# ChocoWu/SeTok

Hardware: AMD Instinct MI355X
Metric: images/s SeTok encode (ViT-L/14, 224^2, dyn-k) (higher is better)
Workload: dtype bf16; 1 GPU; cfg2: ViT-L/14 224^2 (24 of 24 layers, select_layer=-1 as the reference's launch scripts pass it), dyn-k DPC-kNN (k=64, threshold=0.125), SeTok head 1024/2 heads/ff 4096 -> 4096, mm_in_projector mlp2x_gelu; encode-only; batch_per_gpu=256, global_batch=256, slowest_rank=0

## Files before the change

### setok_amd/csrc/common.h

```cpp
#pragma once
#include <hip/hip_runtime.h>
#include <stdint.h>
#include <stdio.h>
#include <stdarg.h>

#include "../../include/setok_hip.h"

#ifdef SETOK_HALF
typedef _Float16 bf16;
typedef __attribute__((ext_vector_type(8))) _Float16 bf16x8;
typedef __attribute__((ext_vector_type(4))) _Float16 bf16x4;
typedef __attribute__((ext_vector_type(2))) _Float16 bf16x2;
#define SETOK_BF16 SETOK_F16
#define __builtin_amdgcn_mfma_f32_16x16x32_bf16 __builtin_amdgcn_mfma_f32_16x16x32_f16
#define __builtin_amdgcn_mfma_f32_32x32x16_bf16 __builtin_amdgcn_mfma_f32_32x32x16_f16
#else
typedef __bf16 bf16;
typedef __attribute__((ext_vector_type(8))) __bf16 bf16x8;
typedef __attribute__((ext_vector_type(4))) __bf16 bf16x4;
typedef __attribute__((ext_vector_type(2))) __bf16 bf16x2;
#endif
typedef __attribute__((ext_vector_type(4))) float f32x4;
typedef __attribute__((ext_vector_type(16))) float f32x16;

// ... 128 lines not shown
    return v;
}

__device__ inline float gelu_erf_fast(float x) {
    const float z = fabsf(x) * 0.70710678118654752440f;
    const float t = __builtin_amdgcn_rcpf(fmaf(0.3275911f, z, 1.0f));
    const float poly = t * fmaf(t, fmaf(t, fmaf(t, fmaf(t, 1.061405429f, -1.453152027f), 1.421413741f), -0.284496736f), 0.254829592f);
    const float half_tail = 0.5f * poly * __builtin_amdgcn_exp2f(-z * z * 1.44269504088896340736f);
    return x * (x >= 0.f ? 1.0f - half_tail : half_tail);
}

__device__ inline unsigned long long dropout_word(unsigned long long seed, unsigned long long group) {
    unsigned long long z = seed + group * 0x9E3779B97F4A7C15ull;
    z = (z ^ (z >> 30)) * 0xBF58476D1CE4E5B9ull;
    z = (z ^ (z >> 27)) * 0x94D049BB133111EBull;
    z ^= z >> 31;
    return z;
}
__device__ inline bool dropout_keep(unsigned long long seed, unsigned long long ctr, unsigned thresh16) {
    return (unsigned)((dropout_word(seed, ctr >> 2) >> (16 * (unsigned)(ctr & 3))) & 0xffffu) >= thresh16;
}


#ifdef SETOK_HALF
__device__ inline void split2(float x, bf16& hi, bf16& lo) {
    hi = (bf16)x;
    lo = (bf16)(x - (float)hi);
}
#else
__device__ inline void split2(float x, bf16& hi, bf16& lo) {
    const unsigned u = __builtin_bit_cast(unsigned, x);
    hi = __builtin_bit_cast(bf16, (unsigned short)(u >> 16));
    const float r = x - __builtin_bit_cast(float, u & 0xffff0000u);
    lo = __builtin_bit_cast(bf16, (unsigned short)(__builtin_bit_cast(unsigned, r) >> 16));
}
#endif
__device__ inline bf16x8 ln_col_frag(float c, float b) {
    bf16x8 f;
#pragma unroll
    for (int e = 0; e < 8; ++e) f[e] = (bf16)0.0f;
    {
        bf16 ch, cl, bh, bl;
        split2(c, ch, cl); split2(b, bh, bl);
        f[0] = ch; f[1] = ch; f[2] = cl; f[3] = cl; f[4] = bh; f[5] = bh; f[6] = bl; f[7] = bl;
    }
    return f;
}
__device__ inline bf16x8 ln_row_frag(float mean, float rstd) {
    bf16x8 f;
#pragma unroll
    for (int e = 0; e < 8; ++e) f[e] = (bf16)0.0f;
    {
        bf16 mh, ml, sh, sl;
        split2(-mean, mh, ml); split2(1.0f / rstd, sh, sl);
        f[0] = mh; f[1] = ml; f[2] = mh; f[3] = ml; f[4] = sh; f[5] = sl; f[6] = sh; f[7] = sl;
    }
    return f;
}

template <typename T>
__device__ inline T swiglu16(float gate, float up) {
    const float g = (float)(T)gate, u = (float)(T)up;
    float s;
    if constexpr (sizeof(T) == 4) s = g / (1.0f + expf(-g));
    else s = g * __builtin_amdgcn_rcpf(1.0f + __builtin_amdgcn_exp2f(-1.44269504088896340736f * g));
    return (T)((float)(T)s * u);
}
constexpr int SETOK_ACT_SWIGLU_PAIRS = 100;

__device__ inline float act_apply(float v, int act) {
    if (act == SETOK_ACT_QUICK_GELU) return v / (1.0f + expf(-1.702f * v));
    if (act == SETOK_ACT_GELU_ERF) return 0.5f * v * (1.0f + erff(v * 0.70710678118654752440f));
    if (act == SETOK_ACT_SILU) return v / (1.0f + expf(-v));
    return v;
}
```

### setok_amd/csrc/gemm_persist.hip

```cpp
#include "lds_mma.h"
#include <stdlib.h>
#include <type_traits>

namespace {

constexpr int TM = 256, TK = 64;
constexpr int STAGE = 64 * 1024;
constexpr int BOFF = TM * TK * 2;

struct PArgs {
    const bf16* A; const bf16* W; const float* bias; const bf16* res; bf16* C;
    int64_t lda, ldc;
    int M, N, K, tilesM, tilesN;
    const float* zero_bias;
    float* Cf;
    int64_t sA, sW, sC;
    int nbatch;
    const float* ln_stats;
    const float* ln_colsum;
    const int32_t* m_dev;
    int rem_rows;
    int rem_tiles;
    int rem_shape;
};

__device__ inline void s_barrier_lgkm() {
    asm volatile("s_waitcnt lgkmcnt(0)\n\ts_barrier" ::: "memory");
}

__device__ inline int swz(int row) { return (row >> 1) & 7; }
typedef __attribute__((ext_vector_type(4))) float f32x4;

__device__ inline bf16x8 ln_frag_lane(const f32x4 raw, int g4) {
    f32x4 v = raw;
    if (g4 != 0) { v[0] = 0.f; v[1] = 0.f; v[2] = 0.f; v[3] = 0.f; }
    return __builtin_bit_cast(bf16x8, v);
}

template <int N_>
__device__ inline void wait_vm() { asm volatile("s_waitcnt vmcnt(%0)" ::"n"(N_) : "memory"); }

constexpr int MAIN_LDS = 2 * STAGE + 8 * 4096;
__device__ float kZeroBias[64];

template <int ACT, bool F32B, bool RESK = false, bool LNK = false>
__global__ __launch_bounds__(512) void gemm_persist_kernel(PArgs g) {
    static_assert(!(LNK && (F32B || RESK)), "the folded LayerNorm feeds qkv / fc1: bf16 out, no residual");
    constexpr int WNC = 4, WR = 128, MI = 4, TNB = 256;
    constexpr int MT = 8, NT = 4;
    constexpr int NL = 8;
    constexpr int NSTORE = WR / 8;
    constexpr int NLN = LNK ? 5 : 0;

    extern __shared__ __attribute__((aligned(16))) char smem[];
    const int tid = threadIdx.x, lane = tid & 63;
    const int wave = __builtin_amdgcn_readfirstlane(tid >> 6);
    const int wm = wave / WNC, wn = wave % WNC;
    const int l15 = lane & 15, g4 = lane >> 4;
    const int nk = g.K / TK;
    const int Mrt = g.m_dev ? min(g.M, __builtin_amdgcn_readfirstlane(*g.m_dev)) : g.M;
    const int tilesMrt = g.m_dev ? (Mrt + TM - 1) / TM : g.tilesM;
    const int tiles_per_problem = tilesMrt * g.tilesN;
    const int num_tiles = tiles_per_problem * (F32B ? g.nbatch : 1);
    const int G = gridDim.x;
    int bz = 0, nbz = 0;

    auto tile_of = [&](int round, int& m0, int& n0, int& b) -> bool {
        int L;
        if ((G & 7) == 0) L = round * G + (blockIdx.x & 7) * (G >> 3) + (blockIdx.x >> 3);
        else L = round * G + blockIdx.x;
        if (L >= num_tiles) return false;
        b = 0;
        if (F32B) { b = L / tiles_per_problem; L -= b * tiles_per_problem; }
        constexpr int GM = 8;
        const int per = GM * g.tilesN, group = L / per, first_m = group * GM;
// ... 12 lines not shown
        b_base = reinterpret_cast<const char*>(Wb_ + (int64_t)n0 * g.K);
        int tid_e = tid;
        asm volatile("" : "+v"(tid_e));
#pragma unroll
        for (int i = 0; i < 4; ++i) {
            const int p = i * 512 + tid_e, row = p >> 3, kc = (p & 7) ^ swz(row);
            a_off[i] = (unsigned)min(row, Mrt - 1 - m0) * (unsigned)(g.lda * 2) + kc * 16;
            b_off[i] = (unsigned)min(row, g.N - 1 - n0) * (unsigned)(g.K * 2) + kc * 16;
        }
    };
    const unsigned lds0 = __builtin_amdgcn_readfirstlane((unsigned)(size_t)(__attribute__((address_space(3))) char*)smem) + wave * 1024;
    auto issue_ktile = [&](int stage, int k0) {
        const unsigned sb = lds0 + stage * STAGE;
#pragma unroll
        for (int i = 0; i < 4; ++i) lds_dma16_sbase(a_base + k0 * 2, a_off[i], sb + i * 8192);
#pragma unroll
        for (int i = 0; i < 4; ++i) lds_dma16_sbase(b_base + k0 * 2, b_off[i], sb + BOFF + i * 8192);
    };

    float nb[NT];
#ifdef SETOK_HALF
    f32x4 nbq[NT];
#endif
    f32x4 ncw; float2 nrw[2];
    float nrs[2], ers[2];
    auto load_bias = [&](int n0_, int m0_) {
        if constexpr (!F32B && !LNK) {
            const float* bp = g.bias ? g.bias + min(n0_ + wn * 64, g.N - 64) : g.zero_bias;
#ifdef SETOK_HALF
#pragma unroll
            for (int j = 0; j < NT; ++j) nbq[j] = *reinterpret_cast<const f32x4*>(bp + (g.bias ? j * 16 + 4 * g4 : 0));
#else
#pragma unroll
            for (int j = 0; j < NT; ++j) nb[j] = bp[j * 16 + l15];
#endif
        }
    };
    auto load_ln_frags = [&](int n0_, int m0_) {
        if constexpr (LNK) {
            ncw = *reinterpret_cast<const f32x4*>(g.ln_colsum + 4 * (int64_t)(min(n0_ + wn * 64, g.N - 64) + g4 * 16 + l15));
#pragma unroll
            for (int i = 0; i < 2; ++i) {
                const float* st = g.ln_stats + 8 * (int64_t)min(m0_ + wm * WR + (2 * g4 + i) * 16 + l15, Mrt - 1);
                nrw[i] = *reinterpret_cast<const float2*>(st);
                nrs[i] = st[4];
            }
        }
    };

    int m0, n0, round = 0;
    if (!tile_of(0, m0, n0, bz)) return;
    set_src(m0, n0, bz);
    load_bias(n0, m0);
    load_ln_frags(n0, m0);
    issue_ktile(0, 0);
    issue_ktile(1, TK);
    int cnt = 0;
    int pend = 0;

    for (;;) {
        int nm0 = 0, nn0 = 0;
        const bool has_next = tile_of(round + 1, nm0, nn0, nbz);

        f32x4 acc[MT][NT];

        auto multiply = [&](auto load_tag, bool do_load, int k_next) {
            constexpr bool LOAD = decltype(load_tag)::value;
            const char* Ab = smem + (cnt & 1) * STAGE;
            const char* Bb = Ab + BOFF;
// ... 19 lines not shown
                    for (int t = 0; t < 4; ++t) {
#pragma unroll
                        for (int j = 0; j < NT; ++j)
                            acc[half * 4 + t][j] = __builtin_amdgcn_mfma_f32_16x16x32_bf16(wf[j], af[t], acc[half * 4 + t][j], 0, 0, 0);
                        if (LOAD && ks == 0) {
                            if (do_load) {
                                __builtin_amdgcn_sched_barrier(0);
                                if (half == 0) lds_dma16_sbase(a_base + k_next * 2, a_off[t], sb + t * 8192);
                                else lds_dma16_sbase(b_base + k_next * 2, b_off[t], sb + BOFF + t * 8192);
                                __builtin_amdgcn_sched_barrier(0);
                            }
                        }
                    }
                    __builtin_amdgcn_s_setprio(0);
                }
            }
            ++cnt;
        };
        using yes = std::true_type; using no = std::false_type;

        if (pend == NSTORE) wait_vm<NSTORE + NL + NLN>(); else wait_vm<NL>();
        s_barrier_lgkm();
        if constexpr (LNK) {
            auto from_group = [&](float v, int grp) {
                return __builtin_bit_cast(float, __builtin_amdgcn_ds_bpermute((l15 + 16 * grp) << 2, __builtin_bit_cast(int, v)));
            };
            bf16x8 cfr[NT];
#pragma unroll
            for (int j = 0; j < NT; ++j) {
                f32x4 v;
#pragma unroll
                for (int e = 0; e < 4; ++e) v[e] = from_group(ncw[e], j);
                cfr[j] = ln_frag_lane(v, g4);
            }
            ers[0] = nrs[0]; ers[1] = nrs[1];
            f32x4 z;
#pragma unroll
            for (int e = 0; e < 4; ++e) z[e] = 0.f;
#pragma unroll
            for (int t = 0; t < MT; ++t) {
                const float d0 = from_group(nrw[t & 1].x, t >> 1), d1 = from_group(nrw[t & 1].y, t >> 1);
                const f32x4 v = {d0, d0, d1, d1};
                const bf16x8 rfr = ln_frag_lane(v, g4);
#pragma unroll
                for (int j = 0; j < NT; ++j) acc[t][j] = __builtin_amdgcn_mfma_f32_16x16x32_bf16(cfr[j], rfr, z, 0, 0, 0);
            }
        } else {
#ifdef SETOK_HALF
            if constexpr (F32B) {
#pragma unroll
                for (int t = 0; t < MT; ++t)
#pragma unroll
                    for (int j = 0; j < NT; ++j) { f32x4 z = {0.f, 0.f, 0.f, 0.f}; acc[t][j] = z; }
            } else {
#pragma unroll
                for (int t = 0; t < MT; ++t)
#pragma unroll
                    for (int j = 0; j < NT; ++j) acc[t][j] = nbq[j];
            }
        }
#else
            bf16x8 ones;
#pragma unroll
            for (int e = 0; e < 8; ++e) ones[e] = (bf16)1.0f;
#pragma unroll
            for (int j = 0; j < NT; ++j) {
                bf16x8 bw;
#pragma unroll
                for (int e = 0; e < 8; ++e) bw[e] = (bf16)0.0f;
// ... 36 lines not shown
        const int64_t wave_elem = (int64_t)(m0 + wm * WR) * g.ldc + (n0 + wn * 64);
        char* c_wave = reinterpret_cast<char*>(g.C + wave_elem);
        const char* r_wave = reinterpret_cast<const char*>(g.res + (RESK ? wave_elem : 0));
        const unsigned lane_off = (unsigned)(lrow * (int)g.ldc + slot * 8) * 2u;
        const unsigned row8 = (unsigned)g.ldc * 16u;
        bf16x8 rv[1][4];
        auto load_residual = [&](auto int_tag, int h) {
#pragma unroll
            for (int it = 0; it < 4; ++it) {
                const int grow = m0 + wm * WR + h * 32 + it * 8 + lrow;
                if (decltype(int_tag)::value || (grow < Mrt && col_ok))
                    rv[0][it] = *reinterpret_cast<const bf16x8*>(r_wave + (size_t)(h * 4 + it) * row8 + lane_off);
            }
        };
        s_barrier_lgkm();
        if (has_next) { set_src(nm0, nn0, nbz); if (!RESK && !LNK) load_bias(nn0, nm0); }
        if (use_res) { if (interior) load_residual(yes{}, 0); else load_residual(no{}, 0); }

        multiply(yes{}, has_next, 0);
        s_barrier_lgkm();
        if (RESK && has_next) load_bias(nn0, nm0);
        auto epilogue = [&](auto res_tag, auto int_tag) {
            constexpr bool RES = decltype(res_tag)::value, INT = decltype(int_tag)::value;
#pragma unroll
            for (int h = 0; h < MI; ++h) {
                float er_pass[2] = {1.f, 1.f};
                if constexpr (LNK) {
#pragma unroll
                    for (int tt = 0; tt < 2; ++tt)
                        er_pass[tt] = __builtin_bit_cast(float, __builtin_amdgcn_ds_bpermute((l15 + 16 * h) << 2, __builtin_bit_cast(int, ers[tt])));
                }
#pragma unroll
                for (int tt = 0; tt < 2; ++tt)
#pragma unroll
                    for (int j = 0; j < NT; ++j) {
                        bf16x4 v;
                        f32x4 xs = acc[2 * h + tt][j];
                        if constexpr (LNK) xs = xs * er_pass[tt];
#pragma unroll
                        for (int e = 0; e < 4; ++e) {
                            float x = xs[e];
                            if (ACT == SETOK_ACT_QUICK_GELU) x = x * __builtin_amdgcn_rcpf(1.0f + __builtin_amdgcn_exp2f(-2.45546696f * x));
                            else if (ACT == SETOK_ACT_GELU_ERF) x = gelu_erf_fast(x);
                            v[e] = (bf16)x;
                        }
                        const int srow = tt * 16 + l15;
                        *reinterpret_cast<bf16x4*>(stg + srow * 128 + (((j * 2 + (g4 >> 1)) ^ (srow & 7)) << 4) + 8 * (g4 & 1)) = v;
                    }
                asm volatile("s_waitcnt lgkmcnt(0)" ::: "memory");
                bf16x8 ov[4];
#pragma unroll
                for (int it = 0; it < 4; ++it) {
                    const int row = it * 8 + lrow;
                    ov[it] = *reinterpret_cast<const bf16x8*>(stg + row * 128 + ((slot ^ (row & 7)) << 4));
                }
                if (RES) {
#pragma unroll
                    for (int it = 0; it < 4; ++it)
#pragma unroll
                        for (int e = 0; e < 8; ++e) ov[it][e] = (bf16)((float)ov[it][e] + (float)rv[0][it][e]);
                }
                if (h == 0) {
                    asm volatile("" ::: "memory");
                    if (has_next) issue_ktile((cnt + 1) & 1, TK);
// ... 39 lines not shown
constexpr int TNS = 8;
__host__ __device__ constexpr int tail_stage(int ttm, int ttn) { return (ttm + ttn) * TK * 2; }
__host__ __device__ constexpr int tail_lds(int ttm, int ttn, int ns) { return ns * tail_stage(ttm, ttn) + 2560; }

template <int ACT, bool LNK, int TTM, int TTN, int NS>
__device__ __forceinline__ void gemm_tail_tile(const PArgs& g, const int tile, char* smem) {
    constexpr int NI = TTM / 32, NJ = TTN / 32;
    constexpr int LPT = NI + NJ;
    constexpr int STG = tail_stage(TTM, TTN);
    static_assert(!LNK || TTM <= 64, "the folded LayerNorm's row values have 64 slots beside the bias row");
    const int tid = threadIdx.x, lane = tid & 63;
    const int wave = __builtin_amdgcn_readfirstlane(tid >> 6);
    const int wm = wave >> 1, wn = wave & 1;
    const int l15 = lane & 15, g4 = lane >> 4;
    const int nk = g.K / TK;
    const int m0 = (tile / g.tilesN) * TTM, n0 = (tile % g.tilesN) * TTN;
    const int Mrt = g.m_dev ? min(g.M, __builtin_amdgcn_readfirstlane(*g.m_dev)) : g.M;
    if (m0 >= Mrt) return;
    float* sbias = reinterpret_cast<float*>(smem + NS * STG);
    if (tid < TTN) sbias[tid] = g.bias ? g.bias[min(n0 + tid, g.N - 1)] : 0.f;
    if constexpr (LNK) {
        if (tid < 64) {
            const float* st = g.ln_stats + 8 * (int64_t)min(m0 + min(tid, TTM - 1), Mrt - 1);
            sbias[64 + tid] = st[4];
            if (tid < TTN) reinterpret_cast<f32x4*>(sbias + 128)[tid] = *reinterpret_cast<const f32x4*>(g.ln_colsum + 4 * (int64_t)min(n0 + tid, g.N - 1));
            const f32x4 rf = {st[0], st[0], st[1], st[1]};
            reinterpret_cast<f32x4*>(sbias + 384)[tid] = rf;
        }
    }

    const bf16* a_src[NI]; const bf16* b_src[NJ];
#pragma unroll
    for (int i = 0; i < NI; ++i) {
        const int p = i * 256 + tid, row = p >> 3, kc = (p & 7) ^ swz(row);
        a_src[i] = g.A + (int64_t)min(m0 + row, Mrt - 1) * g.lda + kc * 8;
    }
#pragma unroll
    for (int i = 0; i < NJ; ++i) {
        const int p = i * 256 + tid, row = p >> 3, kc = (p & 7) ^ swz(row);
        b_src[i] = g.W + (int64_t)min(n0 + row, g.N - 1) * g.K + kc * 8;
    }
    const unsigned lds0 = __builtin_amdgcn_readfirstlane((unsigned)(size_t)(__attribute__((address_space(3))) char*)smem) + wave * 1024;
    auto issue = [&](int kt) {
        const unsigned sb = lds0 + (kt % NS) * STG;
        const int k0 = kt * TK;
#pragma unroll
        for (int i = 0; i < NI; ++i) lds_dma16(a_src[i] + k0, sb + i * 4096);
#pragma unroll
        for (int i = 0; i < NJ; ++i) lds_dma16(b_src[i] + k0, sb + TTM * TK * 2 + i * 4096);
    };
    constexpr bool PAIR = NS >= 6;
    for (int kt = 0; kt < (PAIR ? NS - 2 : NS - 1) && kt < nk; ++kt) issue(kt);

    f32x4 acc[NI][NJ];
    auto init_acc = [&]() {
        if constexpr (LNK) {
            f32x4 z;
#pragma unroll
            for (int e = 0; e < 4; ++e) z[e] = 0.f;
            bf16x8 cfr[NJ];
#pragma unroll
            for (int j = 0; j < NJ; ++j) cfr[j] = ln_frag_lane(reinterpret_cast<const f32x4*>(sbias + 128)[wn * (TTN / 2) + j * 16 + l15], g4);
#pragma unroll
            for (int t = 0; t < NI; ++t) {
                const bf16x8 rfr = ln_frag_lane(reinterpret_cast<const f32x4*>(sbias + 384)[wm * (TTM / 2) + t * 16 + l15], g4);
#pragma unroll
                for (int j = 0; j < NJ; ++j) acc[t][j] = __builtin_amdgcn_mfma_f32_16x16x32_bf16(cfr[j], rfr, z, 0, 0, 0);
            }
        } else {
#pragma unroll
            for (int j = 0; j < NJ; ++j)
#pragma unroll
                for (int e = 0; e < 4; ++e) {
                    const float b = sbias[wn * (TTN / 2) + j * 16 + 4 * g4 + e];
#pragma unroll
                    for (int t = 0; t < NI; ++t) acc[t][j][e] = b;
                }
        }
    };
    auto read_frags = [&](int kt, bf16x8 (&af)[2][NI], bf16x8 (&wf)[2][NJ]) {
        const char* Ab = smem + (kt % NS) * STG;
        const char* Bb = Ab + TTM * TK * 2;
#pragma unroll
        for (int ks = 0; ks < 2; ++ks) {
#pragma unroll
            for (int t = 0; t < NI; ++t) {
                const int ra = wm * (TTM / 2) + t * 16 + l15;
                af[ks][t] = *reinterpret_cast<const bf16x8*>(Ab + ra * 128 + (((ks * 4 + g4) ^ swz(ra)) << 4));
            }
#pragma unroll
            for (int j = 0; j < NJ; ++j) {
// ... 44 lines not shown
                case 2: wait_vm<LPT * 2>(); break;
                case 1: wait_vm<LPT>(); break;
                default: wait_vm<0>(); break;
            }
            s_barrier_lgkm();
            if (kt + NS - 1 < nk) issue(kt + NS - 1);
            if (kt == 0) init_acc();
            bf16x8 af0[2][NI], wf0[2][NJ];
            read_frags(kt, af0, wf0);
            mma_ktile(af0, wf0);
        }
    }
    s_barrier_lgkm();
    char* stg = smem;
    constexpr int RB = TTN * 2, NSL = TTN / 8;
#pragma unroll
    for (int t = 0; t < NI; ++t)
#pragma unroll
        for (int j = 0; j < NJ; ++j) {
            bf16x4 v;
#pragma unroll
            for (int e = 0; e < 4; ++e) {
                float x = acc[t][j][e];
                if constexpr (LNK) x *= sbias[64 + wm * (TTM / 2) + t * 16 + l15];
                if (ACT == SETOK_ACT_QUICK_GELU) x = x * __builtin_amdgcn_rcpf(1.0f + __builtin_amdgcn_exp2f(-2.45546696f * x));
                else if (ACT == SETOK_ACT_GELU_ERF) x = gelu_erf_fast(x);
                v[e] = (bf16)x;
            }
            const int row = wm * (TTM / 2) + t * 16 + l15;
            const int sl = wn * (NSL / 2) + j * 2 + (g4 >> 1);
            *reinterpret_cast<bf16x4*>(stg + row * RB + ((sl ^ (row & (NSL - 1))) << 4) + 8 * (g4 & 1)) = v;
        }
    s_barrier_lgkm();
    const int slot = tid & (NSL - 1), col = n0 + slot * 8;
    constexpr int RPP = 256 / NSL;
    constexpr int PASSES = TTM > RPP ? TTM / RPP : 1;
#pragma unroll
    for (int it = 0; it < PASSES; ++it) {
        const int row = it * RPP + tid / NSL;
        if (row >= TTM) continue;
        const int grow = m0 + row;
        bf16x8 v = *reinterpret_cast<const bf16x8*>(stg + row * RB + ((slot ^ (row & (NSL - 1))) << 4));
        if (grow < Mrt && col < g.N) {
            if (g.res) {
                const bf16x8 rv = *reinterpret_cast<const bf16x8*>(g.res + (int64_t)grow * g.ldc + col);
#pragma unroll
                for (int e = 0; e < 8; ++e) v[e] = (bf16)((float)v[e] + (float)rv[e]);
// ... 64 lines not shown
    else setok_launch(gemm_tail_kernel<2, false, TTM, TTN, NS>, gr, bl, LDS, s, e0, e1, g);
    SETOK_CHECK_LAUNCH("setok_linear(tail)");
    return SETOK_OK;
}

int launch_tail(hipStream_t s, const PArgs& g, int act, hipEvent_t e0, hipEvent_t e1, TailShape sh) {
    if (sh.ttm == 128) return launch_tail_shape<128, 64, 6>(s, g, act, e0, e1);
    if (sh.ttm == 32) return launch_tail_shape<32, 32, TNS>(s, g, act, e0, e1);
    if (sh.ttn == 32) return launch_tail_shape<64, 32, TNS>(s, g, act, e0, e1);
    if (sh.ns == 4) return launch_tail_shape<64, 64, 4>(s, g, act, e0, e1);
    return launch_tail_shape<64, 64, TNS>(s, g, act, e0, e1);
}

#if defined(__HIP_DEVICE_COMPILE__) && !defined(__gfx950__)
#error "gemm_persist.hip is written for gfx950 (MI355X) only: the hand-scheduled waits, hazards and barriers in it are not valid elsewhere"
#endif
template <int ACT, bool LNK, bool RESK, int GRP>
__device__ __forceinline__ void gemm_pp_body(const PArgs& g, char* smem) {
    static_assert(!(LNK && RESK), "the folded LayerNorm feeds q|k|v / fc1: no residual");
    constexpr int QT = 16 * 1024;
    constexpr bool SWG = ACT == SETOK_ACT_SWIGLU_PAIRS;
    static_assert(!(SWG && (LNK || RESK)), "the SwiGLU epilogue has no folded LayerNorm and no residual");
    constexpr int NSTORE = SWG ? 8 : 16;
    constexpr int NAUX = (LNK ? 6 : 4) + (RESK ? 12 : 0);
    const int tid = threadIdx.x, lane = tid & 63;
    const int wave = __builtin_amdgcn_readfirstlane(tid >> 6);
    const int wn = wave & 3;
    const int l15 = lane & 15, g4 = lane >> 4;
    const int nk = g.K / TK;
    const int num_tiles = g.tilesM * g.tilesN;
    const int G = gridDim.x;
    auto tile_of = [&](int round, int& m0, int& n0) -> bool {
        int L;
        if ((G & 7) == 0) L = round * G + (blockIdx.x & 7) * (G >> 3) + (blockIdx.x >> 3);
        else L = round * G + blockIdx.x;
        if (L >= num_tiles) return false;
        constexpr int GM = 8;
        const int per = GM * g.tilesN, group = L / per, first_m = group * GM;
        const int gm = min(g.tilesM - first_m, GM), in = L - group * per;
        m0 = (first_m + in % gm) * TM;
        n0 = (in / gm) * 256;
        return true;
    };
    const int prow = tid >> 3;
    const unsigned kc16 = (unsigned)(((tid & 7) ^ swz(prow)) << 4);
    const unsigned a_off = (unsigned)prow * (unsigned)(g.lda * 2) + kc16;
    const unsigned w_off = (unsigned)prow * (unsigned)(g.K * 2) + kc16;
// ... 37 lines not shown
            dst[t] = *reinterpret_cast<const bf16x8*>(T + r * 128 + (((ks * 4 + g4) ^ swz(r)) << 4));
        }
    };
    auto rd_w = [&](const char* T, int jh, bf16x8 (&dst)[2][2]) {
#pragma unroll
        for (int ks = 0; ks < 2; ++ks)
#pragma unroll
            for (int j = 0; j < 2; ++j) {
                const int r = wn * 64 + jh * 32 + j * 16 + l15;
                dst[ks][j] = *reinterpret_cast<const bf16x8*>(T + BOFF + r * 128 + (((ks * 4 + g4) ^ swz(r)) << 4));
            }
    };
    auto mma8 = [&](int ih, int jh, const bf16x8 (&a)[4], const bf16x8 (&w)[2]) {
#pragma unroll
        for (int t = 0; t < 4; ++t)
#pragma unroll
            for (int j = 0; j < 2; ++j)
                acc[ih * 4 + t][jh * 2 + j] = __builtin_amdgcn_mfma_f32_16x16x32_bf16(w[j], a[t], acc[ih * 4 + t][jh * 2 + j], 0, 0, 0);
    };
    auto lgk0 = [&]() { asm volatile("s_waitcnt lgkmcnt(0)" ::: "memory"); __builtin_amdgcn_sched_barrier(0); };
    auto bar = [&]() { asm volatile("s_barrier" ::: "memory"); };

    f32x4 nbv[4];
    float ers[2];
    f32x4 ncd[4];
    f32x4 npk[2];
    auto ld16 = [&](f32x4& dst, const float* p) { asm volatile("global_load_dwordx4 %0, %1, off" : "=v"(dst) : "v"(p) : "memory"); };
    auto load_start = [&](int n0_, int m0_) {
        if constexpr (LNK) {
#pragma unroll
            for (int j = 0; j < 4; ++j) ld16(ncd[j], g.ln_colsum + 4 * (int64_t)(n0_ + wn * 64 + j * 16 + l15));
#pragma unroll
            for (int i = 0; i < 2; ++i) ld16(npk[i], g.ln_stats + 8 * (int64_t)(m0_ + GRP * 128 + (2 * g4 + i) * 16 + l15));
        } else {
            const float* bp = (g.bias ? g.bias + n0_ : g.zero_bias) + (g.bias ? wn * 64 : 0) + 4 * g4;
#pragma unroll
            for (int j = 0; j < 4; ++j) ld16(nbv[j], bp + (g.bias ? j * 16 : 0));
        }
    };
    constexpr int NBEHIND = NSTORE + (RESK ? 8 : 0);
    auto start_ready = [&]() {
        if constexpr (LNK)
            asm volatile("s_waitcnt vmcnt(%[n])" : "+v"(ncd[0]), "+v"(ncd[1]), "+v"(ncd[2]), "+v"(ncd[3]), "+v"(npk[0]), "+v"(npk[1]) : [n] "n"(NBEHIND) : "memory");
        else
            asm volatile("s_waitcnt vmcnt(%[n])" : "+v"(nbv[0]), "+v"(nbv[1]), "+v"(nbv[2]), "+v"(nbv[3]) : [n] "n"(NBEHIND) : "memory");
    };

    load_start(n0, m0);
    issue_quarter(0, 0); issue_quarter(1, 0); issue_quarter(2, 0); issue_quarter(3, 0); issue_quarter(2, 1); issue_quarter(3, 1);
    asm volatile("s_waitcnt vmcnt(4)" ::: "memory");
    bar();
    int ahead = 0;
    for (;;) {
        start_ready();
        if constexpr (LNK) {
            ers[0] = npk[0][2]; ers[1] = npk[1][2];
            asm volatile("" : "+v"(ers[0]), "+v"(ers[1]));
            f32x4 z;
#pragma unroll
            for (int e = 0; e < 4; ++e) z[e] = 0.f;
#pragma unroll
            for (int t = 0; t < 8; ++t) {
                const bool mine = g4 == (t >> 1);
                const float f0 = mine ? npk[t & 1][0] : 0.f, f1 = mine ? npk[t & 1][1] : 0.f;
                const f32x4 v = {f0, f0, f1, f1};
                const bf16x8 rfr = __builtin_bit_cast(bf16x8, v);
#pragma unroll
                for (int j = 0; j < 4; ++j) acc[t][j] = __builtin_amdgcn_mfma_f32_16x16x32_bf16(__builtin_bit_cast(bf16x8, ncd[j]), rfr, z, 0, 0, 0);
            }
        } else {
#pragma unroll
            for (int t = 0; t < 8; ++t)
#pragma unroll
                for (int j = 0; j < 4; ++j) acc[t][j] = nbv[j];
        }
        if (GRP == 1) bar();
        for (int kt = 0; kt < nk; ++kt) {
            const char* T = smem + ((cnt + kt) & 1) * STAGE;
            const bool skipA = ahead != 0 && kt == 0;
            if (!skipA) { issue_quarter(0, kt + 1); issue_quarter(1, kt + 1); }
            rd_w(T, 0, W0); rd_w(T, 1, W1); rd_a(T, 0, 0, A0[0]); rd_a(T, 0, 1, A0[1]);
            lgk0();
            bar();
            __builtin_amdgcn_s_setprio(1);
            mma8(0, 0, A0[0], W0[0]);
            mma8(0, 0, A0[1], W0[1]);
            mma8(0, 1, A0[0], W1[0]);
            mma8(0, 1, A0[1], W1[1]);
            __builtin_amdgcn_s_setprio(0);
            bar();
            issue_quarter(2, kt + 2); issue_quarter(3, kt + 2);
            rd_a(T, 1, 0, A1[0]); rd_a(T, 1, 1, A1[1]);
// ... 23 lines not shown
                issue_at(1, 1, (cnt + 1) & 1, a_nxt, w_nxt);
            }
        };
        if constexpr (!RESK) issue_next_a1();
        {
            int lane_e = lane;
            asm volatile("" : "+v"(lane_e));
            const int slot = lane_e & 7, lrow = lane_e >> 3;
            char* stg = smem + 2 * STAGE + wave * 4096;
            const int64_t wave_elem = (int64_t)(m0 + GRP * 128) * g.ldc + (SWG ? n0 / 2 + wn * 32 : n0 + wn * 64);
            char* c_wave = reinterpret_cast<char*>(g.C + wave_elem);
            const char* r_wave = reinterpret_cast<const char*>(g.res + (RESK ? wave_elem : 0));
            const unsigned lane_off = SWG ? (unsigned)((lane_e >> 2) * (int)g.ldc + (lane_e & 3) * 8) * 2u : (unsigned)(lrow * (int)g.ldc + slot * 8) * 2u;
            const unsigned row8 = (unsigned)g.ldc * (SWG ? 32u : 16u);
            const unsigned long long c_wave_s = (unsigned long long)(unsigned)__builtin_amdgcn_readfirstlane((int)(unsigned)(unsigned long long)c_wave) |
                                                ((unsigned long long)(unsigned)__builtin_amdgcn_readfirstlane((int)(unsigned)((unsigned long long)c_wave >> 32)) << 32);
            bf16x8 rv[4];
            auto load_residual = [&](int h) {
#pragma unroll
                for (int it = 0; it < 4; ++it) rv[it] = *reinterpret_cast<const bf16x8*>(r_wave + (size_t)(h * 4 + it) * row8 + lane_off);
            };

            if constexpr (RESK) load_residual(0);
#pragma unroll
            for (int h = 0; h < 4; ++h) {
                float er_pass[2] = {1.f, 1.f};
                if constexpr (LNK) {
#pragma unroll
                    for (int tt = 0; tt < 2; ++tt)
                        er_pass[tt] = __builtin_bit_cast(float, __builtin_amdgcn_ds_bpermute((l15 + 16 * h) << 2, __builtin_bit_cast(int, ers[tt])));
                }
#pragma unroll
                for (int tt = 0; tt < 2; ++tt)
#pragma unroll
                    for (int j = 0; j < 4; ++j) {
                        typedef float f32x2 __attribute__((ext_vector_type(2)));
                        typedef bf16 bf16x2 __attribute__((ext_vector_type(2)));
                        bf16x4 v;
                        const f32x4 xq = acc[2 * h + tt][j];
                        if constexpr (SWG) {
                            bf16x2 o2;
                            o2[0] = swiglu16<bf16>(xq[0], xq[1]); o2[1] = swiglu16<bf16>(xq[2], xq[3]);
                            const int srow = tt * 16 + l15;
                            *reinterpret_cast<bf16x2*>(stg + srow * 64 + ((j ^ ((srow >> 1) & 3)) << 4) + 4 * g4) = o2;
                            continue;
                        }
                        if constexpr (ACT == SETOK_ACT_GELU_ERF) {
                            f32x4 xs = xq;
                            if constexpr (LNK) xs = xs * er_pass[tt];
#pragma unroll
                            for (int e = 0; e < 4; ++e) v[e] = (bf16)gelu_erf_fast(xs[e]);
                        } else
#pragma unroll
                        for (int e = 0; e < 4; e += 2) {
                            f32x2 x2 = {xq[e], xq[e + 1]};
                            if constexpr (LNK) x2 = x2 * f32x2{er_pass[tt], er_pass[tt]};
                            if constexpr (ACT == SETOK_ACT_QUICK_GELU) {
                                const f32x2 t = x2 * f32x2{-2.45546696f, -2.45546696f};
                                const f32x2 d = f32x2{__builtin_amdgcn_exp2f(t[0]), __builtin_amdgcn_exp2f(t[1])} + f32x2{1.0f, 1.0f};
                                x2 = x2 * f32x2{__builtin_amdgcn_rcpf(d[0]), __builtin_amdgcn_rcpf(d[1])};
                            }
                            const bf16x2 b2 = __builtin_convertvector(x2, bf16x2);
                            v[e] = b2[0]; v[e + 1] = b2[1];
                        }
                        const int srow = tt * 16 + l15;
                        *reinterpret_cast<bf16x4*>(stg + srow * 128 + (((j * 2 + (g4 >> 1)) ^ (srow & 7)) << 4) + 8 * (g4 & 1)) = v;
                    }
                asm volatile("s_waitcnt lgkmcnt(0)" ::: "memory");
                bf16x8 ov[4];
                if constexpr (SWG) {
#pragma unroll
                    for (int it = 0; it < 2; ++it) {
                        const int row = it * 16 + (lane_e >> 2);
                        ov[it] = *reinterpret_cast<const bf16x8*>(stg + row * 64 + (((lane_e & 3) ^ ((row >> 1) & 3)) << 4));
                    }
                } else {
#pragma unroll
                for (int it = 0; it < 4; ++it) {
                    const int row = it * 8 + lrow;
// ... 203 lines not shown
```

### setok_amd/csrc/norm_attn.hip

```cpp
#include "common.h"

__device__ inline float ln_sq_acc(float x, float mean, float q) {
#pragma clang fp contract(off)
    const float d = x - mean;
    return __builtin_fmaf(d, d, q);
}
__device__ inline float ln_apply(float x, float mean, float rstd, float g, float b) {
#pragma clang fp contract(off)
    const float t = (x - mean) * rstd;
    return __builtin_fmaf(t, g, b);
}

template <typename T>
__global__ __launch_bounds__(256) void layernorm_kernel(const T* x, const float* __restrict__ gamma,
                                                        const float* __restrict__ beta, T* y,
                                                        int rows, int C, float eps, const int32_t* __restrict__ rows_dev) {
    constexpr int V = Elem<T>::VEC;
    const int lane = threadIdx.x & 63;
    const int row = blockIdx.x * 4 + (threadIdx.x >> 6);
    if (rows_dev) rows = min(rows, *rows_dev);
    if (row >= rows) return;
    const T* xr = x + (int64_t)row * C;
    T* yr = y + (int64_t)row * C;
    float buf[V];
// ... 87 lines not shown
    if (dtype == SETOK_BF16 && (C == 512 || C == 768 || C == 1024 || C == 1280 || C == 1536 || C == 2048) && rows >= 1024) {
        if (C == 512) launch_ln_rows<bf16, 1>(s, x, gamma, beta, y, rows, eps, rows_dev);
        else if (C == 768) launch_ln_rows<bf16, 2, 768>(s, x, gamma, beta, y, rows, eps, rows_dev);
        else if (C == 1280) launch_ln_rows<bf16, 3, 1280>(s, x, gamma, beta, y, rows, eps, rows_dev);
        else if (C == 1024) launch_ln_rows<bf16, 2>(s, x, gamma, beta, y, rows, eps, rows_dev);
        else if (C == 1536) launch_ln_rows<bf16, 3>(s, x, gamma, beta, y, rows, eps, rows_dev);
        else launch_ln_rows<bf16, 4>(s, x, gamma, beta, y, rows, eps, rows_dev);
        SETOK_CHECK_LAUNCH("setok_layernorm");
        return SETOK_OK;
    }
    if (dtype == SETOK_BF16) layernorm_kernel<bf16><<<grid, 256, 0, s>>>((const bf16*)x, gamma, beta, (bf16*)y, rows, C, eps, rows_dev);
    else if (dtype == SETOK_F32) layernorm_kernel<float><<<grid, 256, 0, s>>>((const float*)x, gamma, beta, (float*)y, rows, C, eps, rows_dev);
    else return setok_fail(SETOK_EINVAL, "setok_layernorm: bad dtype %d", dtype);
    SETOK_CHECK_LAUNCH("setok_layernorm");
    return SETOK_OK;
}

extern "C" int setok_layernorm(void* stream, int dtype, const void* x, const float* gamma, const float* beta,
                               void* y, int rows, int C, float eps) {
    return setok_layernorm_dev(stream, dtype, x, gamma, beta, y, rows, C, eps, nullptr);
}

__device__ inline void write_row_stats(float* stats, int64_t row, float mean, float rstd) {
    const f32x4 fr = __builtin_bit_cast(f32x4, ln_row_frag(mean, rstd));
    f32x4* o = reinterpret_cast<f32x4*>(stats + 8 * row);
    const f32x4 head = {fr[0], fr[2], rstd, 0.f};
    o[0] = head;
    const f32x4 tail = {rstd, mean, 0.f, 0.f};
    o[1] = tail;
}

template <typename T>
__global__ __launch_bounds__(256) void row_stats_kernel(const T* __restrict__ x, float* __restrict__ stats, int rows, int C, float eps) {
    constexpr int V = Elem<T>::VEC;
    const int lane = threadIdx.x & 63;
    const int wave0 = blockIdx.x * 4 + (threadIdx.x >> 6), nwaves = gridDim.x * 4;
    for (int row = wave0; row < rows; row += nwaves) {
        const T* xr = x + (int64_t)row * C;
        float buf[V];
        float s = 0.f;
        for (int c = lane * V; c < C; c += 64 * V) {
            ld_vec<T>(xr + c, buf);
#pragma unroll
            for (int i = 0; i < V; ++i) s += buf[i];
        }
        const float mean = wave_sum(s) / (float)C;
        float q = 0.f;
        for (int c = lane * V; c < C; c += 64 * V) {
            ld_vec<T>(xr + c, buf);
// ... 58 lines not shown
    else return setok_fail(SETOK_EINVAL, "setok_row_stats: bad dtype %d", dtype);
    SETOK_CHECK_LAUNCH("setok_row_stats");
    return SETOK_OK;
}

__global__ __launch_bounds__(256) void ln_fold_kernel(const bf16* __restrict__ W, const float* __restrict__ gamma, const float* __restrict__ beta,
                                                      const float* __restrict__ bias, bf16* __restrict__ Wg, float* __restrict__ colsum,
                                                      float* __restrict__ bias_folded, float* __restrict__ colfrag, int N, int K) {
    const int lane = threadIdx.x & 63;
    const int n = blockIdx.x * 4 + (threadIdx.x >> 6);
    if (n >= N) return;
    float c = 0.f, bb = 0.f;
    for (int k = lane; k < K; k += 64) {
        const float w = (float)W[(int64_t)n * K + k];
        const bf16 wg = (bf16)(w * gamma[k]);
        Wg[(int64_t)n * K + k] = wg;
        c += (float)wg;
        bb += w * beta[k];
    }
    c = wave_sum(c); bb = wave_sum(bb);
    if (lane == 0) {
        const float bf = (bias ? bias[n] : 0.f) + bb;
        colsum[n] = c; bias_folded[n] = bf;
        reinterpret_cast<f32x4*>(colfrag)[n] = __builtin_bit_cast(f32x4, ln_col_frag(c, bf));
    }
}

extern "C" int setok_ln_fold(void* stream, const void* W, const float* gamma, const float* beta, const float* bias, void* w_gamma,
                             float* w_colsum, float* bias_folded, float* col_frag, int N, int K) {
    SETOK_CHECK_ARG(W && gamma && beta && w_gamma && w_colsum && bias_folded && col_frag && N > 0 && K > 0, "setok_ln_fold: bad argument");
    ln_fold_kernel<<<cdiv(N, 4), 256, 0, (hipStream_t)stream>>>((const bf16*)W, gamma, beta, bias, (bf16*)w_gamma, w_colsum, bias_folded, col_frag, N, K);
    SETOK_CHECK_LAUNCH("setok_ln_fold");
    return SETOK_OK;
}

__device__ inline int attn_rows(const int32_t* seg_offsets, int n_segs, int seg_len, int q_len, int rows, int x, bool key_side, int& r0, int& r1) {
    if (q_len == 0) {
        if (seg_offsets) {
            int lo = 0, hi = n_segs;
            while (hi - lo > 1) { const int mid = (lo + hi) >> 1; if (seg_offsets[mid] <= x) lo = mid; else hi = mid; }
            r0 = seg_offsets[lo]; r1 = seg_offsets[lo + 1];
            if (x >= r1 || x < r0) return -1;
        } else {
            r0 = (x / seg_len) * seg_len; r1 = min(r0 + seg_len, rows);
        }
        return x;
    }
// ... 327 lines not shown
```

Baseline: 6359 images/s.

## Apply folded LayerNorm correction in GEMM epilogue instead of MFMA-seeded accumulators

Replaces the trick of seeding accumulators with MFMA outer products of split-bf16 row/column LayerNorm fragments with zeroed accumulators. The correction is now applied in fp32 in the epilogue as rstd*acc - rstd*mean*colsum + bias. Per-row and per-column stats are parked in LDS once per tile and gathered per lane, which removes the bpermute shuffles and the extra MFMAs. It also reduces the auxiliary global loads. In exchange it adds per-element FMAs and LDS traffic in the epilogue, and it changes the stats/colfrag storage format.

Measured after the change: 6367 images/s, median of 6. No clear change (+0.1%).

```diff
diff --git a/setok_amd/csrc/common.h b/setok_amd/csrc/common.h
--- a/setok_amd/csrc/common.h
+++ b/setok_amd/csrc/common.h
@@ -174,42 +174,6 @@
 }
 
 
-#ifdef SETOK_HALF
-__device__ inline void split2(float x, bf16& hi, bf16& lo) {
-    hi = (bf16)x;
-    lo = (bf16)(x - (float)hi);
-}
-#else
-__device__ inline void split2(float x, bf16& hi, bf16& lo) {
-    const unsigned u = __builtin_bit_cast(unsigned, x);
-    hi = __builtin_bit_cast(bf16, (unsigned short)(u >> 16));
-    const float r = x - __builtin_bit_cast(float, u & 0xffff0000u);
-    lo = __builtin_bit_cast(bf16, (unsigned short)(__builtin_bit_cast(unsigned, r) >> 16));
-}
-#endif
-__device__ inline bf16x8 ln_col_frag(float c, float b) {
-    bf16x8 f;
-#pragma unroll
-    for (int e = 0; e < 8; ++e) f[e] = (bf16)0.0f;
-    {
-        bf16 ch, cl, bh, bl;
-        split2(c, ch, cl); split2(b, bh, bl);
-        f[0] = ch; f[1] = ch; f[2] = cl; f[3] = cl; f[4] = bh; f[5] = bh; f[6] = bl; f[7] = bl;
-    }
-    return f;
-}
-__device__ inline bf16x8 ln_row_frag(float mean, float rstd) {
-    bf16x8 f;
-#pragma unroll
-    for (int e = 0; e < 8; ++e) f[e] = (bf16)0.0f;
-    {
-        bf16 mh, ml, sh, sl;
-        split2(-mean, mh, ml); split2(1.0f / rstd, sh, sl);
-        f[0] = mh; f[1] = ml; f[2] = mh; f[3] = ml; f[4] = sh; f[5] = sl; f[6] = sh; f[7] = sl;
-    }
-    return f;
-}
-
 template <typename T>
 __device__ inline T swiglu16(float gate, float up) {
     const float g = (float)(T)gate, u = (float)(T)up;
diff --git a/setok_amd/csrc/gemm_persist.hip b/setok_amd/csrc/gemm_persist.hip
--- a/setok_amd/csrc/gemm_persist.hip
+++ b/setok_amd/csrc/gemm_persist.hip
@@ -31,10 +31,22 @@
 __device__ inline int swz(int row) { return (row >> 1) & 7; }
 typedef __attribute__((ext_vector_type(4))) float f32x4;
 
-__device__ inline bf16x8 ln_frag_lane(const f32x4 raw, int g4) {
-    f32x4 v = raw;
-    if (g4 != 0) { v[0] = 0.f; v[1] = 0.f; v[2] = 0.f; v[3] = 0.f; }
-    return __builtin_bit_cast(bf16x8, v);
+typedef float f32x2 __attribute__((ext_vector_type(2)));
+__device__ inline float ln_out(float acc, float rstd, float rm, float c, float b) { return __builtin_fmaf(rstd, acc, __builtin_fmaf(-rm, c, b)); }
+__device__ inline f32x2 ln_out2(f32x2 acc, float rstd, float rm, f32x2 c, f32x2 b) {
+    return __builtin_elementwise_fma(f32x2{rstd, rstd}, acc, __builtin_elementwise_fma(f32x2{-rm, -rm}, c, b));
+}
+__device__ inline void ln_park(char* stg, int lane, f32x2 cb, f32x2 r0, f32x2 r1) {
+    float* f = reinterpret_cast<float*>(stg);
+    f[lane] = cb[0]; f[64 + lane] = cb[1];
+    reinterpret_cast<f32x2*>(f + 128)[lane] = r0; reinterpret_cast<f32x2*>(f + 128)[64 + lane] = r1;
+}
+__device__ inline void ln_collect(const char* stg, int l15, int g4, f32x4 (&cq)[4], f32x4 (&bq)[4], f32x2 (&rr)[8]) {
+    const float* f = reinterpret_cast<const float*>(stg);
+#pragma unroll
+    for (int j = 0; j < 4; ++j) { cq[j] = *reinterpret_cast<const f32x4*>(f + j * 16 + 4 * g4); bq[j] = *reinterpret_cast<const f32x4*>(f + 64 + j * 16 + 4 * g4); }
+#pragma unroll
+    for (int t = 0; t < 8; ++t) rr[t] = reinterpret_cast<const f32x2*>(f + 128)[t * 16 + l15];
 }
 
 template <int N_>
@@ -50,7 +62,7 @@
     constexpr int MT = 8, NT = 4;
     constexpr int NL = 8;
     constexpr int NSTORE = WR / 8;
-    constexpr int NLN = LNK ? 5 : 0;
+    constexpr int NLN = LNK ? 3 : 0;
 
     extern __shared__ __attribute__((aligned(16))) char smem[];
     const int tid = threadIdx.x, lane = tid & 63;
@@ -109,8 +121,7 @@
 #ifdef SETOK_HALF
     f32x4 nbq[NT];
 #endif
-    f32x4 ncw; float2 nrw[2];
-    float nrs[2], ers[2];
+    f32x2 ncb, nrs[2];
     auto load_bias = [&](int n0_, int m0_) {
         if constexpr (!F32B && !LNK) {
             const float* bp = g.bias ? g.bias + min(n0_ + wn * 64, g.N - 64) : g.zero_bias;
@@ -125,13 +136,9 @@
     };
     auto load_ln_frags = [&](int n0_, int m0_) {
         if constexpr (LNK) {
-            ncw = *reinterpret_cast<const f32x4*>(g.ln_colsum + 4 * (int64_t)(min(n0_ + wn * 64, g.N - 64) + g4 * 16 + l15));
-#pragma unroll
-            for (int i = 0; i < 2; ++i) {
-                const float* st = g.ln_stats + 8 * (int64_t)min(m0_ + wm * WR + (2 * g4 + i) * 16 + l15, Mrt - 1);
-                nrw[i] = *reinterpret_cast<const float2*>(st);
-                nrs[i] = st[4];
-            }
+            ncb = *reinterpret_cast<const f32x2*>(g.ln_colsum + 4 * (int64_t)(min(n0_ + wn * 64, g.N - 64) + lane));
+#pragma unroll
+            for (int i = 0; i < 2; ++i) nrs[i] = *reinterpret_cast<const f32x2*>(g.ln_stats + 8 * (int64_t)min(m0_ + wm * WR + i * 64 + lane, Mrt - 1));
         }
     };
 
@@ -197,29 +204,11 @@
         if (pend == NSTORE) wait_vm<NSTORE + NL + NLN>(); else wait_vm<NL>();
         s_barrier_lgkm();
         if constexpr (LNK) {
-            auto from_group = [&](float v, int grp) {
-                return __builtin_bit_cast(float, __builtin_amdgcn_ds_bpermute((l15 + 16 * grp) << 2, __builtin_bit_cast(int, v)));
-            };
-            bf16x8 cfr[NT];
-#pragma unroll
-            for (int j = 0; j < NT; ++j) {
-                f32x4 v;
-#pragma unroll
-                for (int e = 0; e < 4; ++e) v[e] = from_group(ncw[e], j);
-                cfr[j] = ln_frag_lane(v, g4);
-            }
-            ers[0] = nrs[0]; ers[1] = nrs[1];
-            f32x4 z;
-#pragma unroll
-            for (int e = 0; e < 4; ++e) z[e] = 0.f;
-#pragma unroll
-            for (int t = 0; t < MT; ++t) {
-                const float d0 = from_group(nrw[t & 1].x, t >> 1), d1 = from_group(nrw[t & 1].y, t >> 1);
-                const f32x4 v = {d0, d0, d1, d1};
-                const bf16x8 rfr = ln_frag_lane(v, g4);
-#pragma unroll
-                for (int j = 0; j < NT; ++j) acc[t][j] = __builtin_amdgcn_mfma_f32_16x16x32_bf16(cfr[j], rfr, z, 0, 0, 0);
-            }
+            ln_park(smem + 2 * STAGE + wave * 4096, lane, ncb, nrs[0], nrs[1]);
+#pragma unroll
+            for (int t = 0; t < MT; ++t)
+#pragma unroll
+                for (int j = 0; j < NT; ++j) { f32x4 z = {0.f, 0.f, 0.f, 0.f}; acc[t][j] = z; }
         } else {
 #ifdef SETOK_HALF
             if constexpr (F32B) {
@@ -302,24 +291,20 @@
         if (RESK && has_next) load_bias(nn0, nm0);
         auto epilogue = [&](auto res_tag, auto int_tag) {
             constexpr bool RES = decltype(res_tag)::value, INT = decltype(int_tag)::value;
+            f32x4 cq[NT], bq[NT]; f32x2 rr[MT];
+            if constexpr (LNK) ln_collect(stg, l15, g4, cq, bq, rr);
 #pragma unroll
             for (int h = 0; h < MI; ++h) {
-                float er_pass[2] = {1.f, 1.f};
-                if constexpr (LNK) {
-#pragma unroll
-                    for (int tt = 0; tt < 2; ++tt)
-                        er_pass[tt] = __builtin_bit_cast(float, __builtin_amdgcn_ds_bpermute((l15 + 16 * h) << 2, __builtin_bit_cast(int, ers[tt])));
-                }
 #pragma unroll
                 for (int tt = 0; tt < 2; ++tt)
 #pragma unroll
                     for (int j = 0; j < NT; ++j) {
                         bf16x4 v;
-                        f32x4 xs = acc[2 * h + tt][j];
-                        if constexpr (LNK) xs = xs * er_pass[tt];
+                        const f32x4 xs = acc[2 * h + tt][j];
 #pragma unroll
                         for (int e = 0; e < 4; ++e) {
                             float x = xs[e];
+                            if constexpr (LNK) x = ln_out(x, rr[2 * h + tt][0], rr[2 * h + tt][1], cq[j][e], bq[j][e]);
                             if (ACT == SETOK_ACT_QUICK_GELU) x = x * __builtin_amdgcn_rcpf(1.0f + __builtin_amdgcn_exp2f(-2.45546696f * x));
                             else if (ACT == SETOK_ACT_GELU_ERF) x = gelu_erf_fast(x);
                             v[e] = (bf16)x;
@@ -405,10 +390,13 @@
     if constexpr (LNK) {
         if (tid < 64) {
             const float* st = g.ln_stats + 8 * (int64_t)min(m0 + min(tid, TTM - 1), Mrt - 1);
-            sbias[64 + tid] = st[4];
-            if (tid < TTN) reinterpret_cast<f32x4*>(sbias + 128)[tid] = *reinterpret_cast<const f32x4*>(g.ln_colsum + 4 * (int64_t)min(n0 + tid, g.N - 1));
-            const f32x4 rf = {st[0], st[0], st[1], st[1]};
-            reinterpret_cast<f32x4*>(sbias + 384)[tid] = rf;
+            sbias[64 + tid] = st[0];
+            sbias[128 + tid] = st[1];
+            if (tid < TTN) {
+                const float* cb = g.ln_colsum + 4 * (int64_t)min(n0 + tid, g.N - 1);
+                sbias[192 + tid] = cb[0];
+                sbias[256 + tid] = cb[1];
+            }
         }
     }
 
@@ -438,18 +426,10 @@
     f32x4 acc[NI][NJ];
     auto init_acc = [&]() {
         if constexpr (LNK) {
-            f32x4 z;
-#pragma unroll
-            for (int e = 0; e < 4; ++e) z[e] = 0.f;
-            bf16x8 cfr[NJ];
-#pragma unroll
-            for (int j = 0; j < NJ; ++j) cfr[j] = ln_frag_lane(reinterpret_cast<const f32x4*>(sbias + 128)[wn * (TTN / 2) + j * 16 + l15], g4);
-#pragma unroll
-            for (int t = 0; t < NI; ++t) {
-                const bf16x8 rfr = ln_frag_lane(reinterpret_cast<const f32x4*>(sbias + 384)[wm * (TTM / 2) + t * 16 + l15], g4);
-#pragma unroll
-                for (int j = 0; j < NJ; ++j) acc[t][j] = __builtin_amdgcn_mfma_f32_16x16x32_bf16(cfr[j], rfr, z, 0, 0, 0);
-            }
+#pragma unroll
+            for (int t = 0; t < NI; ++t)
+#pragma unroll
+                for (int j = 0; j < NJ; ++j) { f32x4 z = {0.f, 0.f, 0.f, 0.f}; acc[t][j] = z; }
         } else {
 #pragma unroll
             for (int j = 0; j < NJ; ++j)
@@ -540,7 +520,10 @@
 #pragma unroll
             for (int e = 0; e < 4; ++e) {
                 float x = acc[t][j][e];
-                if constexpr (LNK) x *= sbias[64 + wm * (TTM / 2) + t * 16 + l15];
+                if constexpr (LNK) {
+                    const int r = wm * (TTM / 2) + t * 16 + l15, c = wn * (TTN / 2) + j * 16 + 4 * g4 + e;
+                    x = ln_out(x, sbias[64 + r], sbias[128 + r], sbias[192 + c], sbias[256 + c]);
+                }
                 if (ACT == SETOK_ACT_QUICK_GELU) x = x * __builtin_amdgcn_rcpf(1.0f + __builtin_amdgcn_exp2f(-2.45546696f * x));
                 else if (ACT == SETOK_ACT_GELU_ERF) x = gelu_erf_fast(x);
                 v[e] = (bf16)x;
@@ -651,7 +634,7 @@
     constexpr bool SWG = ACT == SETOK_ACT_SWIGLU_PAIRS;
     static_assert(!(SWG && (LNK || RESK)), "the SwiGLU epilogue has no folded LayerNorm and no residual");
     constexpr int NSTORE = SWG ? 8 : 16;
-    constexpr int NAUX = (LNK ? 6 : 4) + (RESK ? 12 : 0);
+    constexpr int NAUX = (LNK ? 3 : 4) + (RESK ? 12 : 0);
     const int tid = threadIdx.x, lane = tid & 63;
     const int wave = __builtin_amdgcn_readfirstlane(tid >> 6);
     const int wn = wave & 3;
@@ -735,16 +718,14 @@
     auto bar = [&]() { asm volatile("s_barrier" ::: "memory"); };
 
     f32x4 nbv[4];
-    float ers[2];
-    f32x4 ncd[4];
-    f32x4 npk[2];
+    f32x2 ncb, nrs[2];
     auto ld16 = [&](f32x4& dst, const float* p) { asm volatile("global_load_dwordx4 %0, %1, off" : "=v"(dst) : "v"(p) : "memory"); };
+    auto ld8 = [&](f32x2& dst, const float* p) { asm volatile("global_load_dwordx2 %0, %1, off" : "=v"(dst) : "v"(p) : "memory"); };
     auto load_start = [&](int n0_, int m0_) {
         if constexpr (LNK) {
-#pragma unroll
-            for (int j = 0; j < 4; ++j) ld16(ncd[j], g.ln_colsum + 4 * (int64_t)(n0_ + wn * 64 + j * 16 + l15));
-#pragma unroll
-            for (int i = 0; i < 2; ++i) ld16(npk[i], g.ln_stats + 8 * (int64_t)(m0_ + GRP * 128 + (2 * g4 + i) * 16 + l15));
+            ld8(ncb, g.ln_colsum + 4 * (int64_t)(n0_ + wn * 64 + lane));
+#pragma unroll
+            for (int i = 0; i < 2; ++i) ld8(nrs[i], g.ln_stats + 8 * (int64_t)(m0_ + GRP * 128 + i * 64 + lane));
         } else {
             const float* bp = (g.bias ? g.bias + n0_ : g.zero_bias) + (g.bias ? wn * 64 : 0) + 4 * g4;
 #pragma unroll
@@ -754,7 +735,7 @@
     constexpr int NBEHIND = NSTORE + (RESK ? 8 : 0);
     auto start_ready = [&]() {
         if constexpr (LNK)
-            asm volatile("s_waitcnt vmcnt(%[n])" : "+v"(ncd[0]), "+v"(ncd[1]), "+v"(ncd[2]), "+v"(ncd[3]), "+v"(npk[0]), "+v"(npk[1]) : [n] "n"(NBEHIND) : "memory");
+            asm volatile("s_waitcnt vmcnt(%[n])" : "+v"(ncb), "+v"(nrs[0]), "+v"(nrs[1]) : [n] "n"(NBEHIND) : "memory");
         else
             asm volatile("s_waitcnt vmcnt(%[n])" : "+v"(nbv[0]), "+v"(nbv[1]), "+v"(nbv[2]), "+v"(nbv[3]) : [n] "n"(NBEHIND) : "memory");
     };
@@ -767,20 +748,11 @@
     for (;;) {
         start_ready();
         if constexpr (LNK) {
-            ers[0] = npk[0][2]; ers[1] = npk[1][2];
-            asm volatile("" : "+v"(ers[0]), "+v"(ers[1]));
-            f32x4 z;
-#pragma unroll
-            for (int e = 0; e < 4; ++e) z[e] = 0.f;
-#pragma unroll
-            for (int t = 0; t < 8; ++t) {
-                const bool mine = g4 == (t >> 1);
-                const float f0 = mine ? npk[t & 1][0] : 0.f, f1 = mine ? npk[t & 1][1] : 0.f;
-                const f32x4 v = {f0, f0, f1, f1};
-                const bf16x8 rfr = __builtin_bit_cast(bf16x8, v);
-#pragma unroll
-                for (int j = 0; j < 4; ++j) acc[t][j] = __builtin_amdgcn_mfma_f32_16x16x32_bf16(__builtin_bit_cast(bf16x8, ncd[j]), rfr, z, 0, 0, 0);
-            }
+            ln_park(smem + 2 * STAGE + wave * 4096, lane, ncb, nrs[0], nrs[1]);
+#pragma unroll
+            for (int t = 0; t < 8; ++t)
+#pragma unroll
+                for (int j = 0; j < 4; ++j) { f32x4 z = {0.f, 0.f, 0.f, 0.f}; acc[t][j] = z; }
         } else {
 #pragma unroll
             for (int t = 0; t < 8; ++t)
@@ -850,19 +822,14 @@
             };
 
             if constexpr (RESK) load_residual(0);
+            f32x4 cq[4], bq[4]; f32x2 rr[8];
+            if constexpr (LNK) ln_collect(stg, l15, g4, cq, bq, rr);
 #pragma unroll
             for (int h = 0; h < 4; ++h) {
-                float er_pass[2] = {1.f, 1.f};
-                if constexpr (LNK) {
-#pragma unroll
-                    for (int tt = 0; tt < 2; ++tt)
-                        er_pass[tt] = __builtin_bit_cast(float, __builtin_amdgcn_ds_bpermute((l15 + 16 * h) << 2, __builtin_bit_cast(int, ers[tt])));
-                }
 #pragma unroll
                 for (int tt = 0; tt < 2; ++tt)
 #pragma unroll
                     for (int j = 0; j < 4; ++j) {
-                        typedef float f32x2 __attribute__((ext_vector_type(2)));
                         typedef bf16 bf16x2 __attribute__((ext_vector_type(2)));
                         bf16x4 v;
                         const f32x4 xq = acc[2 * h + tt][j];
@@ -875,14 +842,17 @@
                         }
                         if constexpr (ACT == SETOK_ACT_GELU_ERF) {
                             f32x4 xs = xq;
-                            if constexpr (LNK) xs = xs * er_pass[tt];
+                            if constexpr (LNK) {
+#pragma unroll
+                                for (int e = 0; e < 4; ++e) xs[e] = ln_out(xs[e], rr[2 * h + tt][0], rr[2 * h + tt][1], cq[j][e], bq[j][e]);
+                            }
 #pragma unroll
                             for (int e = 0; e < 4; ++e) v[e] = (bf16)gelu_erf_fast(xs[e]);
                         } else
 #pragma unroll
                         for (int e = 0; e < 4; e += 2) {
                             f32x2 x2 = {xq[e], xq[e + 1]};
-                            if constexpr (LNK) x2 = x2 * f32x2{er_pass[tt], er_pass[tt]};
+                            if constexpr (LNK) x2 = ln_out2(x2, rr[2 * h + tt][0], rr[2 * h + tt][1], f32x2{cq[j][e], cq[j][e + 1]}, f32x2{bq[j][e], bq[j][e + 1]});
                             if constexpr (ACT == SETOK_ACT_QUICK_GELU) {
                                 const f32x2 t = x2 * f32x2{-2.45546696f, -2.45546696f};
                                 const f32x2 d = f32x2{__builtin_amdgcn_exp2f(t[0]), __builtin_amdgcn_exp2f(t[1])} + f32x2{1.0f, 1.0f};
diff --git a/setok_amd/csrc/norm_attn.hip b/setok_amd/csrc/norm_attn.hip
--- a/setok_amd/csrc/norm_attn.hip
+++ b/setok_amd/csrc/norm_attn.hip
@@ -133,9 +133,8 @@
 }
 
 __device__ inline void write_row_stats(float* stats, int64_t row, float mean, float rstd) {
-    const f32x4 fr = __builtin_bit_cast(f32x4, ln_row_frag(mean, rstd));
     f32x4* o = reinterpret_cast<f32x4*>(stats + 8 * row);
-    const f32x4 head = {fr[0], fr[2], rstd, 0.f};
+    const f32x4 head = {rstd, rstd * mean, 0.f, 0.f};
     o[0] = head;
     const f32x4 tail = {rstd, mean, 0.f, 0.f};
     o[1] = tail;
@@ -240,7 +239,8 @@
     if (lane == 0) {
         const float bf = (bias ? bias[n] : 0.f) + bb;
         colsum[n] = c; bias_folded[n] = bf;
-        reinterpret_cast<f32x4*>(colfrag)[n] = __builtin_bit_cast(f32x4, ln_col_frag(c, bf));
+        const f32x4 cb = {c, bf, 0.f, 0.f};
+        reinterpret_cast<f32x4*>(colfrag)[n] = cb;
     }
 }
 
```
